# learner-shx/SVG-IR

Measured on AMD Instinct MI355X. Metric: Gaussian-surfels/sec fwd+bwd @800x800 (1 view), higher is better.
Workload: dtype f32; 1 GPU; cfg2: rgss path, P=200000 surfels, 800x800, SH degree 3, S=5, VS=0, fwd+bwd, one view per step per GPU (BASELINE.json configs[1] = cfg2 at N=1; configs[3] = cfg4, view r on rank r, at N>1); num_rendered=673008, parallelism=view-parallel x1, per_rank_cpus=not pinned

## Files before the change

### svg-ir_amd/csrc/api.hip

```cpp
#include <algorithm>
#include <cstdarg>
#include <cstdio>
#include <atomic>
#include <cstdlib>
#include <ctime>
#include <memory>
#include <mutex>
#include <string>
#include <vector>

#include "common.hpp"
#include "geom_bwd.hpp"
#include "workload_history.hpp"
#include "depth_sort_plan.hpp"

using namespace svgir;

namespace {

thread_local std::string g_err;
std::atomic<bool> g_prof{false};
WorkloadHistory g_history;
unsigned long long* pinned_words(size_t n) {
    void* ptr = nullptr;
// ... 748 lines not shown
        HIP_OK(hipMallocAsync(&redump.p, align_up((size_t)slots * seg_nstate(p->S, ra.VS) * 64 * 4), s));
        ba.seg_state = ra.seg_state = (float*)redump.p;
        g_history.count(WorkloadHistory::kRerunSlots);
        RenderArgs rd = ra;
        rd.slot_cap = (uint32_t)std::min<long long>(slots, 0xffffffffll);
        rd.dump_only = 1;
        rd.queue_order = vc.queue ? 1 : 0;
        if (launch_render_fwd(rd, svgss, s) < 0) return fail(SVGIR_ERR_INVALID, "state re-dump: no specialised composite");
        stage_mark(tm, "state_redump");
        return 0;
    }

    int clears() {
        const size_t need = svgir_backward_scratch_bytes_for(p->variant, p->P, binning_bytes, image_blob, v.W, v.H, p->S, ba.VS);
        if (!generic && (!scratch || scratch_bytes < need))
            return fail(SVGIR_ERR_INVALID, "backward scratch of %zu bytes is smaller than svgir_backward_scratch_bytes_for() = %zu",
                        scratch ? scratch_bytes : (size_t)0, need);
        clear_in_kernel = !generic && R > 0 && g->clear_base && g->clear_bytes && (((uintptr_t)g->clear_base | g->clear_bytes) & 15) == 0;
        ba.clear = clear_in_kernel ? (uint4*)g->clear_base : nullptr;
        ba.clear_n16 = clear_in_kernel ? g->clear_bytes / 16 : 0;
        if (!clear_in_kernel) {
            hipStream_t cs = generic ? s : side_stream(s);
            if (!cs) cs = s;
            hipEvent_t ev_fork = nullptr;
            if (cs != s) {
                HIP_OK(hipEventCreateWithFlags(&ev_fork, hipEventDisableTiming));
                HIP_OK(hipEventRecord(ev_fork, s));
                HIP_OK(hipStreamWaitEvent(cs, ev_fork, 0));
                (void)hipEventDestroy(ev_fork);
            }
            const size_t Pz = (size_t)p->P * 4;
            if (g->clear_base && g->clear_bytes) {
                HIP_OK(hipMemsetAsync(g->clear_base, 0, g->clear_bytes, cs));
            } else {
                struct { float* p; size_t n; } t[] = {
                    {g->dL_dmeans2D, 3 * Pz}, {g->dL_dconic, 4 * Pz}, {g->dL_dopacity, Pz}, {g->dL_dcolors, 3 * Pz},
                    {g->dL_dfeatures, (size_t)p->S * Pz}, {g->dL_dvfeatures, (size_t)ba.VS * Pz}, {g->dL_dnormal, 3 * Pz},
                    {g->dL_ddepth, Pz}, {g->dL_dmeans3D, 3 * Pz}, {g->dL_dcov3D, 6 * Pz}, {g->dL_dsh, (size_t)p->M * 3 * Pz},
                    {g->dL_dscales, 3 * Pz}, {g->dL_drotations, 4 * Pz}, {svgss ? g->dL_dviewmat : nullptr, 64},
                    {svgss ? g->dL_dprojmat : nullptr, 64}, {svgss ? g->dL_dcampos : nullptr, 12}};
                for (auto& e : t)
                    if (e.p && e.n) HIP_OK(hipMemsetAsync(e.p, 0, e.n, cs));
            }
            if (cs != s) {
                HIP_OK(hipEventCreateWithFlags(&cleared.ev, hipEventDisableTiming));
                HIP_OK(hipEventRecord(cleared.ev, cs));
            }
        }
        return 0;
    }

    int seg_build() {
        void* sc_clear = rows ? (void*)ba.row_of : (void*)ba.grad_rows;
        const size_t sc_bytes = rows ? grad_rowof_bytes(caps.cap_R) : align_up((size_t)p->P * grad_row_geom(p->S, ba.VS).RS * 4);
        bool use_list = false;
        if (R > 0) {
            if (p->shade && g->env_grad_work) shade_tabs = shade_tables(&p->shade->sp, g->env_grad_work, p->shade->sp.env_h * p->shade->sp.env_w * 3);
            use_list = g->out_weights && !generic && (p->shade || p->P >= (rows ? kListMinPRows : kListMinP));
            launch_seg_build(ra, sc_clear, sc_bytes, shade_tabs, use_list ? g->out_weights : nullptr, p->P, G.shade_work, s);
        } else if (sc_clear && !rows) {
            HIP_OK(hipMemsetAsync(sc_clear, 0, sc_bytes, s));
        }
        stage_mark(tm, "seg_build");
        if (use_list && R > 0) {
            uint32_t* cnt = G.shade_work + partition_work_words(p->P) - 1;
            launch_partition_scatter(p->P, g->out_weights, G.shade_list, G.shade_work, cnt, s);
            blended = G.shade_list; blended_n = cnt;
        }
        return 0;
    }

    void composite() {
        if (R > 0) {
            if (generic) launch_render_bwd_generic(ba, svgss, s);
            else (void)launch_render_bwd(ba, svgss, s);
        }
        stage_mark(tm, "render_bwd");
        cleared.join();
    }

    void grad_reduce() {
        if (!(R > 0 && rows)) return;
        GradReduceArgs ga;
        ga.list = blended; ga.list_count = blended_n;
        ga.P = p->P; ga.S = p->S; ga.VS = ba.VS; ga.radii = radii; ga.tiles = G.tiles; ga.rec = G.rec;
        ga.grad_rows = ba.grad_rows; ga.row_of = ba.row_of;
        ga.dL_dmean2D = g->dL_dmeans2D; ga.dL_dconic = g->dL_dconic; ga.dL_dopacity = g->dL_dopacity; ga.dL_dcolor = g->dL_dcolors;
        ga.dL_dfeature = g->dL_dfeatures; ga.dL_dvfeature = g->dL_dvfeatures; ga.dL_dnormal = g->dL_dnormal; ga.dL_ddepth = g->dL_ddepth;
        launch_grad_reduce(ga, s);
        stage_mark(tm, "grad_reduce");
    }

    int shade_backward() {
        if (!p->shade) return 0;
        const bool all = p->shade->all_surfels != 0;
        svgir_shade_params sp = p->shade->sp;
        sp.subset = nullptr; sp.subset_count = nullptr;
        if (!all) {
            if (!blended) {
                uint32_t* cnt = G.shade_work + partition_work_words(p->P) - 1;
                launch_partition(p->P, nullptr, g->out_weights, G.shade_list, G.shade_work, cnt, s);
                blended = G.shade_list; blended_n = cnt;
            }
            sp.subset = blended; sp.subset_count = blended_n;
        }
        auto in_clear = [&](const float* t, size_t floats) {
            const char* b = (const char*)g->clear_base, *q = (const char*)t;
// ... 22 lines not shown
        ga.dL_dopacity = g->dL_dopacity; ga.dL_dfeature = g->dL_dfeatures;
        ga.dL_dmean3D = g->dL_dmeans3D; ga.dL_dcov3D = g->dL_dcov3D; ga.dL_dsh = g->dL_dsh; ga.dL_dscale = g->dL_dscales;
        ga.dL_drot = g->dL_drotations; ga.dL_dviewmat = g->dL_dviewmat; ga.dL_dprojmat = g->dL_dprojmat; ga.dL_dcampos = g->dL_dcampos;
        if (ga.scales && !ga.rotations) return fail(SVGIR_ERR_INVALID, "rotations missing");
        launch_geom_bwd_blended(ga, g->out_weights, s);
        stage_mark(tm, "geom_bwd");
        hipError_t e = p->debug ? hipStreamSynchronize(s) : hipSuccess;
        if (e == hipSuccess) e = hipGetLastError();
        return e != hipSuccess ? fail(SVGIR_ERR_HIP, "backward failed: %s", hipGetErrorString(e)) : 0;
    }
};

int svgir_forward(const svgir_params* p, const svgir_outputs* o, svgir_alloc_fn geom, void* geom_ctx,
                  svgir_alloc_fn binning, void* binning_ctx, svgir_alloc_fn image, void* image_ctx, void* stream) {
    return ForwardCall::run({p, o, geom, geom_ctx, binning, binning_ctx, image, image_ctx, stream, 0}, true);
}

int svgir_forward_batch(svgir_view_call* views, int32_t count) {
    if (count < 0 || (count > 0 && !views)) return fail(SVGIR_ERR_INVALID, "views is NULL");
    std::vector<std::unique_ptr<ForwardCall>> calls;
    calls.reserve((size_t)count);
    int first_err = 0;
    for (int v = 0; v < count; v++) {
        calls.emplace_back(new ForwardCall(views[v], true));
        const int rc = calls.back()->begin();
        views[v].num_rendered = rc < 0 ? rc : 0;
        if (rc < 0 && !first_err) first_err = rc;
    }
    const std::string begin_err = first_err ? g_err : std::string();
    for (int v = 0; v < count; v++) {
        if (views[v].num_rendered < 0) continue;
        const int rc = calls[(size_t)v]->finish();
        views[v].num_rendered = rc;
        if (rc < 0 && !first_err) first_err = rc;
    }
    if (!begin_err.empty()) g_err = begin_err;
    return first_err;
}
void svgir_reset_workload_history(int32_t scope) { g_history.reset(scope); }
void svgir_speculation_stats(int64_t* out5) {
    if (out5) g_history.stats(out5);
}

size_t svgir_backward_scratch_bytes(int32_t variant, int32_t P, size_t binning_bytes, int32_t W, int32_t H, int32_t S,
                                    int32_t VS) {
    return svgir_backward_scratch_bytes_for(variant, P, binning_bytes, nullptr, W, H, S, VS);
}

size_t svgir_backward_scratch_bytes_for(int32_t variant, int32_t P, size_t binning_bytes, const char* image_blob, int32_t W, int32_t H,
                                        int32_t S, int32_t VS) {
    if (!render_specialised(S, variant == SVGIR_SVGSS ? VS : 0, variant == SVGIR_SVGSS))
        return 256;
    if (variant != SVGIR_SVGSS || VS == 0)
        return align_up((size_t)(P > 0 ? P : 1) * grad_row_geom(S, 0).RS * 4);
    ViewCounts vc;
    if (!bin_capacity(binning_bytes, image_blob, W, H, seg_nstate(S, VS), Wait::kBlock, nullptr, &vc))
        vc.cap_R = binning_capacity((long long)(binning_bytes / 48));
    if (image_blob && vc.pairs < 0) (void)hipGetLastError();
    const size_t rows = vc.pairs >= 0 ? (size_t)std::min<long long>(vc.pairs, (long long)4 * vc.cap_R) : (size_t)4 * vc.cap_R;
    return grad_scratch_bytes(vc.cap_R, rows > 0 ? rows : 1, S, VS);
}

int svgir_backward(const svgir_params* p, const svgir_grads* g, int32_t R, const int32_t* radii, char* geom_blob,
                   char* binning_blob, size_t binning_bytes, char* image_blob, char* scratch, size_t scratch_bytes,
                   void* stream) {
    return BackwardCall{p, g, R, radii, geom_blob, binning_blob, binning_bytes, image_blob, scratch, scratch_bytes, (hipStream_t)stream}.run();
}

int svgir_mark_visible(int32_t variant, int32_t P, const float* means3D, const float* viewmatrix,
                       const float* projmatrix, uint8_t* present, void* stream) {
    (void)projmatrix;
    if (P < 0) return fail(SVGIR_ERR_INVALID, "P < 0");
    if (P == 0 || variant == SVGIR_SVGSS) return 0;
    if (!means3D || !viewmatrix || !present) return fail(SVGIR_ERR_INVALID, "NULL pointer");
    launch_mark_visible(P, means3D, viewmatrix, present, (hipStream_t)stream);
    hipError_t e = hipGetLastError();
    if (e != hipSuccess) return fail(SVGIR_ERR_HIP, "mark_visible failed: %s", hipGetErrorString(e));
    return 0;
}

}
```

### svg-ir_amd/csrc/common.hpp

```cpp
#pragma once
#include <hip/hip_runtime.h>
#include <stddef.h>
#include <stdint.h>
#include <stdlib.h>

#include <algorithm>

#include "../../include/svgir_raster.h"
#include "wave.hpp"

namespace svgir {

constexpr int TILE = 16;
constexpr int BLOCK = 256;
constexpr int REC = 24;

enum RecField {
    R_X = 0, R_Y = 1, R_CX = 2, R_CY = 3,
    R_CZ = 4, R_OP = 5, R_DEPTH = 6, R_DA = 7,
    R_J0 = 8, R_J1 = 9, R_J2 = 10, R_J3 = 11,
    R_DB = 12, R_R = 13, R_G = 14, R_B = 15,
    R_NX = 16, R_NY = 17, R_NZ = 18, R_IU = 19,
    R_IV = 20, R_IBASE = 21, R_RECT = 22, R_PAD2 = 23
};
// ... 99 lines not shown

constexpr int SEG_CLASSES = 5, SEG_BLOCK_STRIDE = 8;

struct ImageLayout {
    float* final_T;
    float* final_D;
    int32_t* n_contrib;
    uint32_t* ranges;
    uint32_t* seg_block;
    uint32_t* sub_total;
    uint32_t* sub_order;
    uint32_t* sub_count;
    uint32_t* sub_ndump;
    uint32_t* sub_pair_base;
    uint32_t* sub_slot_base;
    uint32_t* counters;
    uint32_t* disp_ctr;
    uint32_t* disp_item;
    size_t ncontrib_off;
    size_t bytes;
};
constexpr int DISP_NCLS = 64, DISP_SHARDS = 8, DISP_STEP = 16;
constexpr int DISP_CTR_WORDS = DISP_NCLS * DISP_SHARDS + 2;
inline ImageLayout image_layout(char* base, int W, int H) {
    ImageLayout im;
    size_t off = 0;
    auto take = [&](size_t bytes) { char* p = base ? base + off : nullptr; off += align_up(bytes); return p; };
    const size_t N = (size_t)W * H;
    const size_t T = (size_t)((W + TILE - 1) / TILE) * ((H + TILE - 1) / TILE);
    im.final_T = (float*)take(N * 4);
    im.final_D = (float*)take(N * 4);
    im.ncontrib_off = off;
    im.n_contrib = (int32_t*)take(N * 4);
    im.ranges = (uint32_t*)take((T * 2 + (T + 255) / 256 * SEG_BLOCK_STRIDE) * 4);
    im.seg_block = im.ranges ? im.ranges + T * 2 : nullptr;
    im.sub_total = (uint32_t*)take(T * 4 * 4);
    im.sub_order = (uint32_t*)take(order_entries((W + TILE - 1) / TILE, (H + TILE - 1) / TILE) * 4);
    im.sub_count = (uint32_t*)take(T * 4 * 4);
    im.sub_ndump = (uint32_t*)take(T * 4 * 4);
    im.sub_pair_base = (uint32_t*)take(T * 4 * 4);
    im.sub_slot_base = (uint32_t*)take(T * 4 * 4);
    im.counters = (uint32_t*)take(32);
    im.disp_ctr = (uint32_t*)take(DISP_CTR_WORDS * 4);
    im.disp_item = (uint32_t*)take(order_entries((W + TILE - 1) / TILE, (H + TILE - 1) / TILE) * DISP_NCLS * 4);
    im.bytes = off;
    return im;
}

struct GradRowGeom { int NC0, P4, VS, GEO, RS; };
inline GradRowGeom grad_row_geom(int S, int VS) {
    GradRowGeom g;
    g.NC0 = 7 + S; g.P4 = (g.NC0 + 3) / 4 * 4; g.VS = VS; g.GEO = g.P4 + VS; g.RS = (g.GEO + 6 + 3) / 4 * 4;
    return g;
}
inline size_t grad_rowof_bytes(int cap) { return align_up((size_t)4 * cap * 4); }
inline size_t grad_scratch_bytes(int cap, size_t rows, int S, int VS) {
    return grad_rowof_bytes(cap) + align_up(rows * grad_row_geom(S, VS).RS * 4);
}

constexpr int SEG = 64;
#if defined(__HIPCC__)
__host__ __device__
#endif
inline uint32_t seg_slots(uint32_t total) { return total >= (uint32_t)SEG ? total / (uint32_t)SEG + 1u : 0u; }
inline size_t seg_capacity(int R, int T) { return (size_t)4 * (size_t)(R > 0 ? R : 0) / SEG + (size_t)4 * T + 1; }
constexpr int SEG_K_BITS = 14;
struct SegDesc { uint32_t sm, r0, len, count, ndump, pair_base, slot_base, pad2; };
#if defined(__HIPCC__)
__host__ __device__
#endif
inline int seg_class(uint32_t nent) { return nent >= (uint32_t)SEG ? 0 : 4 - (int)(nent * 4u / (uint32_t)SEG); }
#ifndef SEG_XCD_BLOCK_V
#define SEG_XCD_BLOCK_V 32
#endif
constexpr uint32_t SEG_XCD_BLOCK = SEG_XCD_BLOCK_V;
#if defined(__HIPCC__)
__host__ __device__
#endif
inline uint32_t seg_item_of(uint32_t w) {
    const uint32_t c = w & 7u, q = w >> 3;
    return ((q / SEG_XCD_BLOCK) * 8u + c) * SEG_XCD_BLOCK + (q % SEG_XCD_BLOCK);
}
#if defined(__HIPCC__)
__host__ __device__
#endif
inline uint32_t seg_work_ids(uint32_t n) { return (n + 8u * SEG_XCD_BLOCK - 1u) / (8u * SEG_XCD_BLOCK) * (8u * SEG_XCD_BLOCK); }

inline int binning_capacity(long long R) {
    const long long c = ((R > 0 ? R : 1) + 4095) / 4096 * 4096;
    return (int)(c > 0x7ffff000LL ? 0x7ffff000LL : c);
}

struct TileSortPlan { int bits, passes, bits_per_pass; bool single; };
constexpr int TS12_BINS = 4096, TS12_KEYS = 2048;
inline bool tile_sort_single_enabled() {
    static const bool on = [] { const char* e = getenv("SVGIR_TILE_SORT12"); return !(e && e[0] == '0'); }();
    return on;
}
inline TileSortPlan tile_sort_plan(int T) {
    int bits = 1;
    while ((1 << bits) < T) bits++;
    TileSortPlan p;
    p.bits = bits;
    p.single = T <= TS12_BINS && tile_sort_single_enabled();
    p.passes = p.single ? 1 : (bits + 7) / 8;
    p.bits_per_pass = p.single ? bits : (bits + p.passes - 1) / p.passes;
// ... 321 lines not shown
```

### svg-ir_amd/csrc/geom_bwd.hip

```cpp
#include "common.hpp"
#include "geom_bwd.hpp"

#pragma clang fp contract(off)

namespace svgir {

namespace {

struct Mat3 {
    float m[3][3];
};
__device__ __forceinline__ Mat3 mmul(const Mat3& A, const Mat3& B) {
    Mat3 r;
#pragma unroll
    for (int c = 0; c < 3; c++)
#pragma unroll
        for (int row = 0; row < 3; row++)
            r.m[c][row] = A.m[0][row] * B.m[c][0] + A.m[1][row] * B.m[c][1] + A.m[2][row] * B.m[c][2];
    return r;
}
__device__ __forceinline__ Mat3 mtr(const Mat3& A) {
    Mat3 r;
#pragma unroll
    for (int c = 0; c < 3; c++)
// ... 20 lines not shown
    int total = 0;
    {
        int cand[CHUNKS];
        bool take[CHUNKS];
#pragma unroll
        for (int c = 0; c < CHUNKS; c++) {
            const int w = blockIdx.x * GB_SPAN + c * GB_BLOCK + lane;
            const bool in_range = w < n;
            cand[c] = in_range ? (a.list ? (int)a.list[w] : w) : 0;
            take[c] = in_range && (by_weight ? weights[cand[c]] > 0.f : a.radii[cand[c]] > 0);
        }
#pragma unroll
        for (int c = 0; c < CHUNKS; c++) {
            const unsigned long long m = __ballot(take[c]);
            if (take[c]) sIdx[total + __popcll(m & ((lane == 0) ? 0ull : (~0ull >> (64 - lane))))] = cand[c];
            total += __popcll(m);
        }
    }
    if (total == 0) return;
    const bool vec = a.shs && a.M == 16 && ((((size_t)a.shs) | ((size_t)a.dL_dsh)) & 15) == 0;
    const bool coop = vec && a.D == 3;
    const int rsub = lane / 12, rpart = lane - rsub * 12;
    wave_lds_sync();
    const int npass = CHUNKS == 1 ? 1 : (total + GB_BLOCK - 1) / GB_BLOCK;
    for (int p0 = 0; p0 < npass * GB_BLOCK; p0 += GB_BLOCK) {
        const int nvis = min(GB_BLOCK, total - p0);
        const bool visible = lane < nvis;
        const int idx = visible ? sIdx[p0 + lane] : 0;
        const int* sI = sIdx + p0;
        constexpr int CR = 6;
        float4 cr[CR];
        if (coop) {
    #pragma unroll
            for (int j = 0; j < CR; j++) {
                const int r = 5 * j + rsub;
                cr[j] = (rsub < 5 && r < nvis) ? reinterpret_cast<const float4*>(a.shs)[(size_t)sI[r] * 12 + rpart]
                                              : make_float4(0.f, 0.f, 0.f, 0.f);
            }
        }
        const bool surface = cfg_flag(a.cfg, 0);
        const bool lrn_cam = a.svgss && a.cfg.len >= 0 && cfg_flag(a.cfg, 3);
        float V[16], PR[16], campos[3] = {0.f, 0.f, 0.f};
        float in_color[3] = {0.f, 0.f, 0.f}, in_normal[3] = {0.f, 0.f, 0.f}, in_depth = 0.f, in_m2d[2] = {0.f, 0.f}, in_conic[3] = {0.f, 0.f, 0.f}, in_opacity = 0.f;
        float mean[3] = {0.f, 0.f, 0.f}, c3[6] = {0.f, 0.f, 0.f, 0.f, 0.f, 0.f};
        float4 qq = make_float4(0.f, 0.f, 0.f, 0.f);
        float sc_in[3] = {0.f, 0.f, 0.f};
        uint32_t cm = 0;
        if (visible) {
    #pragma unroll
        for (int i = 0; i < 16; i++) { V[i] = a.view[i]; PR[i] = a.proj[i]; }
        if (a.shs) { campos[0] = a.campos[0]; campos[1] = a.campos[1]; campos[2] = a.campos[2]; }

        if (a.packed) {
            const int P4 = (7 + a.S + 3) / 4 * 4, RS = (P4 + 6 + 3) / 4 * 4;
            const float* row = a.packed + (size_t)idx * RS;
            const float4 h0 = reinterpret_cast<const float4*>(row)[0], h1 = reinterpret_cast<const float4*>(row)[1];
            const float4 t0 = reinterpret_cast<const float4*>(row + P4)[0], t1 = reinterpret_cast<const float4*>(row + P4)[1];
            in_color[0] = h0.x; in_color[1] = h0.y; in_color[2] = h0.z; in_normal[0] = h0.w; in_normal[1] = h1.x; in_normal[2] = h1.y;
            in_depth = h1.z;
            in_m2d[0] = t0.x; in_m2d[1] = t0.y; in_conic[0] = t0.z; in_conic[1] = t0.w; in_conic[2] = t1.x;
            in_opacity = t1.y;
        } else {
    #pragma unroll
            for (int c = 0; c < 3; c++) { in_color[c] = a.dL_dcolor[3 * idx + c]; in_normal[c] = a.dL_dnormal[3 * idx + c]; }
            in_depth = a.dL_ddepth[idx];
            in_m2d[0] = a.dL_dmean2D[3 * idx]; in_m2d[1] = a.dL_dmean2D[3 * idx + 1];
            in_conic[0] = a.dL_dconic[4 * idx]; in_conic[1] = a.dL_dconic[4 * idx + 1]; in_conic[2] = a.dL_dconic[4 * idx + 3];
        }
        mean[0] = a.means3D[3 * idx]; mean[1] = a.means3D[3 * idx + 1]; mean[2] = a.means3D[3 * idx + 2];
    #pragma unroll
        for (int i = 0; i < 6; i++) c3[i] = a.cov3D[6 * idx + i];
        if (a.shs) cm = a.clamped[idx];
        if (a.scales) {
            qq = reinterpret_cast<const float4*>(a.rotations)[idx];
    #pragma unroll
            for (int i = 0; i < 3; i++) sc_in[i] = a.scales[3 * idx + i];
        }
        }
        if (coop) {
    #pragma unroll
            for (int j = 0; j < CR; j++) {
                const int r = 5 * j + rsub;
                if (rsub < 5 && r < nvis) sRow[r][rpart] = cr[j];
            }
            for (int r0 = 5 * CR; r0 < nvis; r0 += 5) {
                const int r = r0 + rsub;
                if (rsub < 5 && r < nvis)
                    sRow[r][rpart] = reinterpret_cast<const float4*>(a.shs)[(size_t)sI[r] * 12 + rpart];
            }
        }
        if (visible) {
        const int nk = (a.D + 1) * (a.D + 1);
        float sh[48];
        if (a.shs) {
            const float* shp = a.shs + (size_t)idx * a.M * 3;
            if (coop) {
                wave_lds_sync();
    #pragma unroll
                for (int i = 0; i < 12; i++) {
                    const float4 v = sRow[lane][i];
                    sh[4 * i] = v.x; sh[4 * i + 1] = v.y; sh[4 * i + 2] = v.z; sh[4 * i + 3] = v.w;
                }
            } else if (vec) {
    #pragma unroll
                for (int i = 0; i < 12; i++) {
                    const float4 v = reinterpret_cast<const float4*>(shp)[i];
                    sh[4 * i] = v.x; sh[4 * i + 1] = v.y; sh[4 * i + 2] = v.z; sh[4 * i + 3] = v.w;
                }
            } else {
    #pragma unroll
                for (int i = 0; i < 48; i++) sh[i] = i < 3 * nk ? shp[i] : 0.f;
            }
        }
        if (a.packed) {
            const int P4 = (7 + a.S + 3) / 4 * 4, RS = (P4 + 6 + 3) / 4 * 4;
            const float* row = a.packed + (size_t)idx * RS;
            for (int c = 0; c < a.S; c++) a.dL_dfeature[(size_t)idx * a.S + c] = row[7 + c];
        }
        float dmean[3];
        float dcv[6];

        {
            const float dcon[3] = {in_conic[0], in_conic[1], in_conic[2]};
            float t[3] = {V[0] * mean[0] + V[4] * mean[1] + V[8] * mean[2] + V[12],
                          V[1] * mean[0] + V[5] * mean[1] + V[9] * mean[2] + V[13],
                          V[2] * mean[0] + V[6] * mean[1] + V[10] * mean[2] + V[14]};
            const float limx = 1.3f * a.tanx, limy = 1.3f * a.tany;
            const float txtz = t[0] / t[2], tytz = t[1] / t[2];
            t[0] = fminf(limx, fmaxf(-limx, txtz)) * t[2];
            t[1] = fminf(limy, fmaxf(-limy, tytz)) * t[2];
            const float xgm = (txtz < -limx || txtz > limx) ? 0.f : 1.f;
            const float ygm = (tytz < -limy || tytz > limy) ? 0.f : 1.f;
            const float hx = a.focal_x, hy = a.focal_y;
            const float J0 = hx / t[2], J1 = -(hx * t[0]) / (t[2] * t[2]), J2 = hy / t[2], J3 = -(hy * t[1]) / (t[2] * t[2]);
            Mat3 Jm, Wm, Vk;
            Jm.m[0][0] = J0; Jm.m[0][1] = 0.f; Jm.m[0][2] = J1;
            Jm.m[1][0] = 0.f; Jm.m[1][1] = J2; Jm.m[1][2] = J3;
            Jm.m[2][0] = 0.f; Jm.m[2][1] = 0.f; Jm.m[2][2] = 0.f;
            Wm.m[0][0] = V[0]; Wm.m[0][1] = V[4]; Wm.m[0][2] = V[8];
            Wm.m[1][0] = V[1]; Wm.m[1][1] = V[5]; Wm.m[1][2] = V[9];
            Wm.m[2][0] = V[2]; Wm.m[2][1] = V[6]; Wm.m[2][2] = V[10];
            Vk.m[0][0] = c3[0]; Vk.m[0][1] = c3[1]; Vk.m[0][2] = c3[2];
            Vk.m[1][0] = c3[1]; Vk.m[1][1] = c3[3]; Vk.m[1][2] = c3[4];
            Vk.m[2][0] = c3[2]; Vk.m[2][1] = c3[4]; Vk.m[2][2] = c3[5];
            const Mat3 Tm = mmul(Wm, Jm);
            const Mat3 cov = mmul(mmul(mtr(Tm), mtr(Vk)), Tm);
            const float ca = cov.m[0][0] + 0.3f, cb = cov.m[0][1], cc = cov.m[1][1] + 0.3f;
            const float denom = ca * cc - cb * cb;
            float da = 0.f, db = 0.f, dc = 0.f;
            const float d2i = 1.0f / ((denom * denom) + 0.0000001f);
    #define TC(i, j) Tm.m[i][j]
    #define VC_(i, j) Vk.m[i][j]
            if (d2i != 0) {
                da = d2i * (-cc * cc * dcon[0] + 2 * cb * cc * dcon[1] + (denom - ca * cc) * dcon[2]);
                dc = d2i * (-ca * ca * dcon[2] + 2 * ca * cb * dcon[1] + (denom - ca * cc) * dcon[0]);
                db = d2i * 2 * (cb * cc * dcon[0] - (denom + 2 * cb * cb) * dcon[1] + ca * cb * dcon[2]);
                dcv[0] = (TC(0, 0) * TC(0, 0) * da + TC(0, 0) * TC(1, 0) * db + TC(1, 0) * TC(1, 0) * dc);
                dcv[3] = (TC(0, 1) * TC(0, 1) * da + TC(0, 1) * TC(1, 1) * db + TC(1, 1) * TC(1, 1) * dc);
                dcv[5] = (TC(0, 2) * TC(0, 2) * da + TC(0, 2) * TC(1, 2) * db + TC(1, 2) * TC(1, 2) * dc);
                dcv[1] = 2 * TC(0, 0) * TC(0, 1) * da + (TC(0, 0) * TC(1, 1) + TC(0, 1) * TC(1, 0)) * db + 2 * TC(1, 0) * TC(1, 1) * dc;
                dcv[2] = 2 * TC(0, 0) * TC(0, 2) * da + (TC(0, 0) * TC(1, 2) + TC(0, 2) * TC(1, 0)) * db + 2 * TC(1, 0) * TC(1, 2) * dc;
                dcv[4] = 2 * TC(0, 2) * TC(0, 1) * da + (TC(0, 1) * TC(1, 2) + TC(0, 2) * TC(1, 1)) * db + 2 * TC(1, 1) * TC(1, 2) * dc;
            } else {
    #pragma unroll
                for (int i = 0; i < 6; i++) dcv[i] = 0.f;
            }
            const float dT00 = 2 * (TC(0, 0) * VC_(0, 0) + TC(0, 1) * VC_(0, 1) + TC(0, 2) * VC_(0, 2)) * da +
                               (TC(1, 0) * VC_(0, 0) + TC(1, 1) * VC_(0, 1) + TC(1, 2) * VC_(0, 2)) * db;
            const float dT01 = 2 * (TC(0, 0) * VC_(1, 0) + TC(0, 1) * VC_(1, 1) + TC(0, 2) * VC_(1, 2)) * da +
// ... 221 lines not shown
```

### svg-ir_amd/csrc/render_bwd_plain.hip

```cpp
#include <algorithm>

#include "common.hpp"
#include "stage.hpp"
#include "dev_trace.hpp"

namespace svgir {

namespace {

typedef const __attribute__((address_space(4))) float cfloat;
typedef const __attribute__((address_space(4))) uint32_t cuint;

#ifndef BWDP_GRID_MULT
#define BWDP_GRID_MULT 4
#endif
#ifndef BWDP_WPE
#define BWDP_WPE 4
#endif

template <int S>
struct PlainGeom {
    static constexpr int SB = 8;
    static constexpr int NC0 = 7 + S;
    static constexpr int GROW = NC0 + 1;
    static constexpr int PS = 68;
    static constexpr int PROWS = 24;
    static constexpr size_t off_m = (size_t)PROWS * PS * 4;
    static constexpr size_t off_c = off_m + (size_t)SB * 8 * 4;
    static constexpr size_t off_q = off_c + (size_t)3 * SB * 16;
    static constexpr size_t lds_bytes = off_q + (size_t)SEG * 8;
    static_assert(NC0 <= 16, "one 16-wide MFMA column tile");
    static_assert((size_t)64 * GROW * 4 <= off_m, "the G transposition tile aliases the panel");
};

template <int S, bool SVGSS>
__global__ void __launch_bounds__(64) __attribute__((amdgpu_waves_per_eu(BWDP_WPE, BWDP_WPE)))
render_bwd_plain_kernel(const RenderBwdArgs a) {
    using PG = PlainGeom<S>;
    constexpr int SB = PG::SB, NC0 = PG::NC0, GROW = PG::GROW, PS = PG::PS;
    constexpr int SS = S > 0 ? S : 1;
    constexpr int P4 = (NC0 + 3) / 4 * 4, GEO = P4, RS = (GEO + 6 + 3) / 4 * 4;
    extern __shared__ __attribute__((aligned(16))) char smem[];
    float* sP = reinterpret_cast<float*>(smem);
    float* sG = sP;
    float* sM = reinterpret_cast<float*>(smem + PG::off_m);
    float4* sC = reinterpret_cast<float4*>(smem + PG::off_c);
    uint2* sQ = reinterpret_cast<uint2*>(smem + PG::off_q);

    const int lane = threadIdx.x;
    const bool surface = cfg_flag(a.cfg, 0), normalize_depth = cfg_flag(a.cfg, 1);
    const bool sp = surface && cfg_flag(a.cfg, 2);
    const bool bgeom = SVGSS ? true : (a.backward_geometry != 0);
    const size_t N_ = (size_t)a.W * a.H;
    const float ddelx_dx = 0.5f * a.W, ddely_dy = 0.5f * a.H;
    const int colB = lane & 15, grpB = lane >> 4;

    float cx0, cx1, cx2, momy[2];
    {
        const int ex = colB == 1 || colB == 4 ? 1 : colB == 3 ? 2 : 0;
        const int ey = colB == 2 || colB == 4 ? 1 : colB == 5 ? 2 : 0;
        cx0 = (colB < 6 && ex == 0) ? 1.f : 0.f; cx1 = ex == 1 ? 1.f : 0.f; cx2 = ex == 2 ? 1.f : 0.f;
#pragma unroll
        for (int h = 0; h < 2; h++) {
            const float my = (float)(2 * grpB + h) - 3.5f;
            momy[h] = ey == 0 ? 1.f : ey == 1 ? my : my * my;
        }
    }

    typedef const __attribute__((address_space(4))) uint32_t cu32;
    cu32* dsc0 = (cu32*)(uintptr_t)(a.seg_desc + min(seg_item_of(blockIdx.x), (uint32_t)a.seg_cap));
    uint32_t d_sm = dsc0[0], d_r0 = dsc0[1], d_len = dsc0[2], d_count = dsc0[3], d_ndump = dsc0[4], d_sb = dsc0[6];
    if (a.clear) {
        const uint4 z = make_uint4(0u, 0u, 0u, 0u);
        for (size_t i = (size_t)blockIdx.x * 64 + threadIdx.x; i < a.clear_n16; i += (size_t)gridDim.x * 64) a.clear[i] = z;
    }
    const uint32_t nlive = min(a.seg_count[0], (uint32_t)a.seg_cap);
    const uint32_t nwork = seg_work_ids(nlive);
    if (blockIdx.x >= nwork) return;
    DEV_TRACE_DECL();
    [[maybe_unused]] unsigned dev_items = 0, dev_cands = 0;
    for (uint32_t w = blockIdx.x; w < nwork; w += gridDim.x) {
    const uint32_t item = seg_item_of(w);
    if (item >= nlive) continue;
    if (w != blockIdx.x) {
        cu32* dsc = (cu32*)(uintptr_t)(a.seg_desc + item);
        d_sm = dsc[0]; d_r0 = dsc[1]; d_len = dsc[2]; d_count = dsc[3]; d_ndump = dsc[4]; d_sb = dsc[6];
    }
    wave_lds_sync();
    const uint32_t sm = d_sm, r0 = d_r0, tlen = d_len;
    const int count = (int)d_count, ndump = (int)d_ndump;
    const int sid = (int)(sm >> SEG_K_BITS), kseg = (int)(sm & ((1u << SEG_K_BITS) - 1u));
    const int tile = sid >> 2, sub = sid & 3;
    const int seg_lo = kseg * SEG, seg_hi = min(count, seg_lo + SEG);
    if (seg_hi <= seg_lo) continue;
// ... 57 lines not shown
    for (int i = 0; i < 3; i++) { gC[i] = (inside && a.g_color) ? a.g_color[i * N_ + pid] : 0.f; gN[i] = (inside && a.g_normal) ? a.g_normal[i * N_ + pid] : 0.f; }
#pragma unroll
    for (int i = 0; i < SS; i++) gF[i] = (inside && i < S && a.g_feature) ? a.g_feature[i * N_ + pid] : 0.f;
    if (inside) { gD = a.g_depth ? a.g_depth[pid] : 0.f; gO = a.g_opacity ? a.g_opacity[pid] : 0.f; }
    const float bgdot = a.bg[0] * gC[0] + a.bg[1] * gC[1] + a.bg[2] * gC[2];
    const float omt = 1.f - T_final;
    const float gDn = normalize_depth ? gD / omt : gD;
    const float kdn = normalize_depth ? -gD * D_final * T_final / (omt * omt) : 0.f;
    const float gO_kbg = gO - (bgdot + (normalize_depth ? 0.f : 10.f * gD));
    const float q5g = sp ? -gD : 0.f;

    uint32_t wmax = last_contributor;
    wmax = wave_reduce_max(wmax);
    if (wmax == 0) continue;

    float T = T_final;
    float last_alpha = 0.f;
    float A_acc = 0.f, s_last = 0.f;
    if (kseg < ndump) {
        constexpr int NST = 8 + S;
        const uint32_t sbase = d_sb;
        const float* e = a.seg_state + ((size_t)(sbase + kseg) * NST) * 64 + lane;
        const float* f = a.seg_state + ((size_t)(sbase + ndump) * NST) * 64 + lane;
        T = e[0];
        float dot = (f[7 * 64] - e[7 * 64]) * gDn;
#pragma unroll
        for (int i = 0; i < 3; i++) {
            dot += (f[(1 + i) * 64] - e[(1 + i) * 64]) * gC[i];
            dot += (f[(4 + i) * 64] - e[(4 + i) * 64]) * gN[i];
        }
        if (bgeom) {
#pragma unroll
            for (int i = 0; i < S; i++) dot += (f[(8 + i) * 64] - e[(8 + i) * 64]) * gF[i];
        }
        A_acc = dot * __builtin_amdgcn_rcpf(T);
    }

    {
        float* g = sG + lane * GROW;
        g[0] = gC[0]; g[1] = gC[1]; g[2] = gC[2];
        g[3] = surface ? gN[0] * 10.f : 0.f; g[4] = surface ? gN[1] * 10.f : 0.f; g[5] = surface ? gN[2] * 10.f : 0.f;
        g[6] = gDn;
#pragma unroll
        for (int i = 0; i < S; i++) g[7 + i] = gF[i];
    }
    float Bp[16];
    wave_lds_sync();
    {
        const float* gB = sG + (16 * grpB) * GROW + (colB < NC0 ? colB : 0);
#pragma unroll
        for (int kk = 0; kk < 16; kk++) Bp[kk] = colB < NC0 ? gB[kk * GROW] : 0.f;
    }
    wave_lds_sync();

    int nskip = 0;
    {
        uint2 e = make_uint2(0u, 0u);
        if (lane < nent) e = sub_in[seg_hi - 1 - lane];
        sQ[lane] = e;
        nskip = __popcll(__ballot(lane < nent && e.y >= wmax));
    }
    const float gNe0 = surface ? gN[0] : 0.f, gNe1 = surface ? gN[1] : 0.f, gNe2 = surface ? gN[2] : 0.f;
    float gFe[SS];
#pragma unroll
    for (int i = 0; i < SS; i++) gFe[i] = bgeom ? gF[i] : 0.f;
    const float spf = sp ? 1.f : 0.f;
    const float gOT = gO_kbg * T_final;

    const int cstart = (nskip / SB) * SB;
    Cand cur = spec_cur;
    Entry en1 = spec_en1;
    if (cstart != 0) {
        cur = fetch_rec(fetch_entry(cstart));
        en1 = fetch_entry(cstart + 1);
    }
    auto prefetch_consts = [&](int cb) {
        int lC = lane;
        asm volatile("" : "+v"(lC));
        if (lC < 3 * SB) {
            const int cq = lC & 7, chunk = lC >> 3;
            const uint32_t gq = sQ[min(cb + cq, SEG - 1)].x;
            const float* src = a.rec + (uint32_t)(gq * (uint32_t)REC + (uint32_t)(chunk == 2 ? 12 : 4 * chunk));
            __builtin_amdgcn_global_load_lds(src, (__attribute__((address_space(3))) void*)(smem + PG::off_c), 16, 0, 0);
        }
    };
    wave_lds_sync();
    prefetch_consts(cstart);
    DEV_TRACE_MARK(0);
    dev_items++; dev_cands += (unsigned)nent;
    for (int c0 = cstart; c0 < nent; c0 += SB) {
        uint32_t live = 0;
        float hw = 0.f, hv = 0.f, hu = 0.f;
#pragma unroll
        for (int k = 0; k < SB; k++) {
            const Cand nxt = fetch_rec(en1);
            en1 = fetch_entry(c0 + k + 2);
            const float dx = cur.X - pxf, dy = cur.Y - pyf;
            if (k > 0) {
                sP[(k - 1) * PS + lane] = hw; sP[(SB + k - 1) * PS + lane] = hv; sP[(2 * SB + k - 1) * PS + lane] = hu;
            }
            const float pw = pair_power(cur.cxx, cur.cxy, cur.cyy, dx, dy);
            const float Gs = exp_nonpos(pw);
            const float al = fminf(0.99f, cur.op * Gs);
            const bool pre = cur.slot < last_contributor && pw <= 0.0f && al >= (1.0f / 255.0f);
            const float ioma = __builtin_amdgcn_rcpf(1.f - al);
            float sd = cur.cr * gC[0] + cur.cg * gC[1] + cur.cb * gC[2];
            sd += cur.nx * gNe0 + cur.ny * gNe1 + cur.nz * gNe2;
            const float d_cur = cur.dep - spf * (dx * cur.DA + dy * cur.DB);
            sd += d_cur * gDn;
#pragma unroll
            for (int ch = 0; ch < S; ch++) sd += cur.f[ch] * gFe[ch];
            const float inv_Told = __builtin_amdgcn_rcpf(T);
            const float Tn = T * ioma;
            const float An = last_alpha * s_last + (1.f - last_alpha) * A_acc;
            float dL_dalpha = kdn * inv_Told + (sd - An);
            dL_dalpha *= Tn;
            dL_dalpha += gOT * ioma;
            T = pre ? Tn : T;
            A_acc = pre ? An : A_acc;
            s_last = pre ? sd : s_last;
            last_alpha = pre ? al : last_alpha;
            hw = pre ? al * Tn : 0.f;
            hv = pre ? Gs * dL_dalpha : 0.f;
            hu = pre ? q5g : 0.f;
            live |= (__builtin_amdgcn_ballot_w64(pre) != 0ull ? 1u : 0u) << k;
            cur = nxt;
        }
        sP[(SB - 1) * PS + lane] = hw; sP[(2 * SB - 1) * PS + lane] = hv; sP[(3 * SB - 1) * PS + lane] = hu;
        DEV_TRACE_MARK(2);
        if (live != 0) {
        wave_lds_sync();
        int lB = lane;
        asm volatile("" : "+v"(lB));
        const int colB = lB & 15, grpB = lB >> 4;
        f32x4 accM = {0.f, 0.f, 0.f, 0.f};
        {
            const float4* ap = reinterpret_cast<const float4*>(sP + (SB + colB) * PS + 16 * grpB);
            const float4 a0 = ap[0], a1 = ap[1], a2 = ap[2], a3 = ap[3];
            const float av[16] = {a0.x, a0.y, a0.z, a0.w, a1.x, a1.y, a1.z, a1.w,
                                  a2.x, a2.y, a2.z, a2.w, a3.x, a3.y, a3.z, a3.w};
            float c0l = cx0;
            asm volatile("" : "+v"(c0l));
#pragma unroll
            for (int kk = 0; kk < 16; kk++) {
                const float mx = (float)(kk & 7) - 3.5f;
                accM = __builtin_amdgcn_mfma_f32_16x16x4f32(av[kk], (c0l + mx * (cx1 + mx * cx2)) * momy[kk >> 3], accM, 0, 0, 0);
            }
        }
        if (grpB < 2) {
            if (colB < 6) {
#pragma unroll
                for (int rr = 0; rr < 4; rr++) sM[(4 * grpB + rr) * 8 + colB] = accM[rr];
            }
        } else if (colB == 0) {
#pragma unroll
            for (int rr = 0; rr < 4; rr++) sM[(4 * (grpB - 2) + rr) * 8 + 6] = accM[rr];
        }
        f32x4 accP = {0.f, 0.f, 0.f, 0.f};
        {
            const float4* ap = reinterpret_cast<const float4*>(sP + colB * PS + 16 * grpB);
            const float4 a0 = ap[0], a1 = ap[1], a2 = ap[2], a3 = ap[3];
            const float av[16] = {a0.x, a0.y, a0.z, a0.w, a1.x, a1.y, a1.z, a1.w,
                                  a2.x, a2.y, a2.z, a2.w, a3.x, a3.y, a3.z, a3.w};
#pragma unroll
            for (int kk = 0; kk < 16; kk++) accP = __builtin_amdgcn_mfma_f32_16x16x4f32(av[kk], Bp[kk], accP, 0, 0, 0);
        }
        __builtin_amdgcn_s_waitcnt(0x0f70);
        wave_lds_sync();
        DEV_TRACE_MARK(3);
        {
            const int cq = lB & 7, jq = lB >> 3;
            if (jq < 6 && ((live >> cq) & 1u)) {
                const float4 m03 = *reinterpret_cast<const float4*>(sM + cq * 8);
                const float4 m47 = *reinterpret_cast<const float4*>(sM + cq * 8 + 4);
                const float4 Aq = sC[cq], Bq = sC[SB + cq];
                const float DBq = sC[2 * SB + cq].x;
                const float Xc = Aq.x - cxs, Yc = Aq.y - cys;
                const float M0 = m03.x, M1 = m03.y, M2 = m03.z, M3 = m03.w, M4 = m47.x, M5 = m47.y, Q = m47.z;
                const float Sx = Xc * M0 - M1, Sy = Yc * M0 - M2;
                const float hf = Bq.y * -0.5f;
                float ge;
                if (jq == 0) ge = hf * 2.f * (Aq.z * Sx + Aq.w * Sy) * ddelx_dx + Q * Bq.w;
                else if (jq == 1) ge = hf * 2.f * (Bq.x * Sy + Aq.w * Sx) * ddely_dy + Q * DBq;
                else if (jq == 2) ge = hf * (Xc * (Sx - M1) + M3);
                else if (jq == 3) ge = hf * ((Xc * Sy - Yc * M1) + M4);
                else if (jq == 4) ge = hf * (Yc * (Sy - M2) + M5);
                else ge = M0;
                if (ge != 0.f) atomic_add_f32(a.grad_rows + (uint32_t)(sQ[c0 + cq].x * (uint32_t)RS + (uint32_t)(GEO + jq)), ge);
            }
        }
        if (grpB < 2) {
#pragma unroll
            for (int rr = 0; rr < 4; rr++) {
                const int cB = 4 * grpB + rr;
                const bool mine = ((live >> cB) & 1u) && colB < NC0 && accP[rr] != 0.f;
                if (mine) atomic_add_f32(a.grad_rows + (uint32_t)(sQ[c0 + cB].x * (uint32_t)RS + (uint32_t)colB), accP[rr]);
            }
        }
        wave_lds_sync();
        }
        if (c0 + SB < nent) prefetch_consts(c0 + SB);
        DEV_TRACE_MARK(1);
    }
    }
    DEV_TRACE_END(1, dev_items, dev_cands, blockIdx.x);
}

template <int S, bool SVGSS>
void launch(const RenderBwdArgs& a, hipStream_t s) {
    using PG = PlainGeom<S>;
    const int grid = std::max(8, std::min(a.seg_cap, BWDP_GRID_MULT * 256 * 4 * BWDP_WPE) & ~7);
    hipLaunchKernelGGL((render_bwd_plain_kernel<S, SVGSS>), dim3(grid), dim3(64), PG::lds_bytes, s, a);
}

}

int launch_render_bwd_plain(const RenderBwdArgs& a, bool svgss, hipStream_t s) {
    if (a.VS != 0) return -1;
#define CASE(SV, SG) if (a.S == SV && svgss == SG) { launch<SV, SG>(a, s); return 0; }
    CASE(0, true) CASE(5, true) CASE(0, false) CASE(5, false) CASE(3, false) CASE(1, false)
#undef CASE
    return -1;
}

#if defined(SVGIR_DEV)
extern "C" int svgir_dev_trace_read_bwd_plain(unsigned long long* out, int cap_records) {
    unsigned int n[2];
    if (hipMemcpyFromSymbol(n, HIP_SYMBOL(svgir::g_dev_trace_n), sizeof(n)) != hipSuccess) return -1;
    int cnt = (int)std::min<unsigned>(n[1], (unsigned)std::min(cap_records, svgir::DEV_TRACE_CAP));
    if (cnt > 0 && hipMemcpyFromSymbol(out, HIP_SYMBOL(svgir::g_dev_trace), (size_t)cnt * svgir::DEV_TRACE_WORDS * 8,
                                       (size_t)svgir::DEV_TRACE_CAP * svgir::DEV_TRACE_WORDS * 8) != hipSuccess) return -1;
    n[1] = 0;
    (void)hipMemcpyToSymbol(HIP_SYMBOL(svgir::g_dev_trace_n), n, sizeof(n));
    return cnt;
}
#endif

}
```

Measured before the change: 630.4 million surfels/s.

## Batch color-gradient MFMA over two segment chunks and centralize packed row geometry

The color/feature gradient MFMA in the plain backward render kernel now runs once per pair of SB-sized chunks. It double-buffers the weight rows in LDS (PROWS raised from 24 to 32) and tracks a combined 16-bit liveness mask, so all 16 MFMA rows do useful work instead of half being padding. This cuts MFMA issues, LDS reads and sync points per chunk, in exchange for more LDS and extra zeroing of the second buffer. It also adds a packed_row_geom helper with an optional 16/32 alignment mode (off by default) and an optional split-accumulator MFMA variant (off by default).

```diff
diff --git a/svg-ir_amd/csrc/api.hip b/svg-ir_amd/csrc/api.hip
--- a/svg-ir_amd/csrc/api.hip
+++ b/svg-ir_amd/csrc/api.hip
@@ -824,7 +824,7 @@
 
     int seg_build() {
         void* sc_clear = rows ? (void*)ba.row_of : (void*)ba.grad_rows;
-        const size_t sc_bytes = rows ? grad_rowof_bytes(caps.cap_R) : align_up((size_t)p->P * grad_row_geom(p->S, ba.VS).RS * 4);
+        const size_t sc_bytes = rows ? grad_rowof_bytes(caps.cap_R) : align_up((size_t)p->P * packed_row_geom(p->S).RS * 4);
         bool use_list = false;
         if (R > 0) {
             if (p->shade && g->env_grad_work) shade_tabs = shade_tables(&p->shade->sp, g->env_grad_work, p->shade->sp.env_h * p->shade->sp.env_w * 3);
@@ -953,7 +953,7 @@
     if (!render_specialised(S, variant == SVGIR_SVGSS ? VS : 0, variant == SVGIR_SVGSS))
         return 256;
     if (variant != SVGIR_SVGSS || VS == 0)
-        return align_up((size_t)(P > 0 ? P : 1) * grad_row_geom(S, 0).RS * 4);
+        return align_up((size_t)(P > 0 ? P : 1) * packed_row_geom(S).RS * 4);
     ViewCounts vc;
     if (!bin_capacity(binning_bytes, image_blob, W, H, seg_nstate(S, VS), Wait::kBlock, nullptr, &vc))
         vc.cap_R = binning_capacity((long long)(binning_bytes / 48));
diff --git a/svg-ir_amd/csrc/common.hpp b/svg-ir_amd/csrc/common.hpp
--- a/svg-ir_amd/csrc/common.hpp
+++ b/svg-ir_amd/csrc/common.hpp
@@ -175,6 +175,14 @@
     GradRowGeom g;
     g.NC0 = 7 + S; g.P4 = (g.NC0 + 3) / 4 * 4; g.VS = VS; g.GEO = g.P4 + VS; g.RS = (g.GEO + 6 + 3) / 4 * 4;
     return g;
+}
+#ifndef PACKED_ROW_ALIGNED
+#define PACKED_ROW_ALIGNED 0
+#endif
+struct PackedRowGeom { int NC0, GEO, RS; };
+constexpr PackedRowGeom packed_row_geom(int S) {
+    const int NC0 = 7 + S, P4 = (NC0 + 3) / 4 * 4, RC = (P4 + 6 + 3) / 4 * 4;
+    return (!PACKED_ROW_ALIGNED || RC <= 16 || P4 > 16) ? PackedRowGeom{NC0, P4, RC} : PackedRowGeom{NC0, 16, 32};
 }
 inline size_t grad_rowof_bytes(int cap) { return align_up((size_t)4 * cap * 4); }
 inline size_t grad_scratch_bytes(int cap, size_t rows, int S, int VS) {
diff --git a/svg-ir_amd/csrc/geom_bwd.hip b/svg-ir_amd/csrc/geom_bwd.hip
--- a/svg-ir_amd/csrc/geom_bwd.hip
+++ b/svg-ir_amd/csrc/geom_bwd.hip
@@ -96,10 +96,10 @@
         if (a.shs) { campos[0] = a.campos[0]; campos[1] = a.campos[1]; campos[2] = a.campos[2]; }
 
         if (a.packed) {
-            const int P4 = (7 + a.S + 3) / 4 * 4, RS = (P4 + 6 + 3) / 4 * 4;
-            const float* row = a.packed + (size_t)idx * RS;
+            const PackedRowGeom rg = packed_row_geom(a.S);
+            const float* row = a.packed + (size_t)idx * rg.RS;
             const float4 h0 = reinterpret_cast<const float4*>(row)[0], h1 = reinterpret_cast<const float4*>(row)[1];
-            const float4 t0 = reinterpret_cast<const float4*>(row + P4)[0], t1 = reinterpret_cast<const float4*>(row + P4)[1];
+            const float4 t0 = reinterpret_cast<const float4*>(row + rg.GEO)[0], t1 = reinterpret_cast<const float4*>(row + rg.GEO)[1];
             in_color[0] = h0.x; in_color[1] = h0.y; in_color[2] = h0.z; in_normal[0] = h0.w; in_normal[1] = h1.x; in_normal[2] = h1.y;
             in_depth = h1.z;
             in_m2d[0] = t0.x; in_m2d[1] = t0.y; in_conic[0] = t0.z; in_conic[1] = t0.w; in_conic[2] = t1.x;
@@ -157,8 +157,7 @@
             }
         }
         if (a.packed) {
-            const int P4 = (7 + a.S + 3) / 4 * 4, RS = (P4 + 6 + 3) / 4 * 4;
-            const float* row = a.packed + (size_t)idx * RS;
+            const float* row = a.packed + (size_t)idx * packed_row_geom(a.S).RS;
             for (int c = 0; c < a.S; c++) a.dL_dfeature[(size_t)idx * a.S + c] = row[7 + c];
         }
         float dmean[3];
diff --git a/svg-ir_amd/csrc/render_bwd_plain.hip b/svg-ir_amd/csrc/render_bwd_plain.hip
--- a/svg-ir_amd/csrc/render_bwd_plain.hip
+++ b/svg-ir_amd/csrc/render_bwd_plain.hip
@@ -17,6 +17,9 @@
 #ifndef BWDP_WPE
 #define BWDP_WPE 4
 #endif
+#ifndef BWDP_MFMA_ACC
+#define BWDP_MFMA_ACC 1
+#endif
 
 template <int S>
 struct PlainGeom {
@@ -24,7 +27,7 @@
     static constexpr int NC0 = 7 + S;
     static constexpr int GROW = NC0 + 1;
     static constexpr int PS = 68;
-    static constexpr int PROWS = 24;
+    static constexpr int PROWS = 32;
     static constexpr size_t off_m = (size_t)PROWS * PS * 4;
     static constexpr size_t off_c = off_m + (size_t)SB * 8 * 4;
     static constexpr size_t off_q = off_c + (size_t)3 * SB * 16;
@@ -39,7 +42,7 @@
     using PG = PlainGeom<S>;
     constexpr int SB = PG::SB, NC0 = PG::NC0, GROW = PG::GROW, PS = PG::PS;
     constexpr int SS = S > 0 ? S : 1;
-    constexpr int P4 = (NC0 + 3) / 4 * 4, GEO = P4, RS = (GEO + 6 + 3) / 4 * 4;
+    constexpr int GEO = packed_row_geom(S).GEO, RS = packed_row_geom(S).RS;
     extern __shared__ __attribute__((aligned(16))) char smem[];
     float* sP = reinterpret_cast<float*>(smem);
     float* sG = sP;
@@ -203,6 +206,8 @@
         for (int kk = 0; kk < 16; kk++) Bp[kk] = colB < NC0 ? gB[kk * GROW] : 0.f;
     }
     wave_lds_sync();
+#pragma unroll
+    for (int k = 0; k < SB; k++) sP[(SB + k) * PS + lane] = 0.f;
 
     int nskip = 0;
     {
@@ -239,7 +244,10 @@
     prefetch_consts(cstart);
     DEV_TRACE_MARK(0);
     dev_items++; dev_cands += (unsigned)nent;
+    uint32_t live16 = 0;
     for (int c0 = cstart; c0 < nent; c0 += SB) {
+        const int par = ((c0 - cstart) / SB) & 1;
+        float* sPw = sP + par * (SB * PS) + lane;
         uint32_t live = 0;
         float hw = 0.f, hv = 0.f, hu = 0.f;
 #pragma unroll
@@ -248,7 +256,7 @@
             en1 = fetch_entry(c0 + k + 2);
             const float dx = cur.X - pxf, dy = cur.Y - pyf;
             if (k > 0) {
-                sP[(k - 1) * PS + lane] = hw; sP[(SB + k - 1) * PS + lane] = hv; sP[(2 * SB + k - 1) * PS + lane] = hu;
+                sPw[(k - 1) * PS] = hw; sP[(2 * SB + k - 1) * PS + lane] = hv; sP[(3 * SB + k - 1) * PS + lane] = hu;
             }
             const float pw = pair_power(cur.cxx, cur.cxy, cur.cyy, dx, dy);
             const float Gs = exp_nonpos(pw);
@@ -277,7 +285,7 @@
             live |= (__builtin_amdgcn_ballot_w64(pre) != 0ull ? 1u : 0u) << k;
             cur = nxt;
         }
-        sP[(SB - 1) * PS + lane] = hw; sP[(2 * SB - 1) * PS + lane] = hv; sP[(3 * SB - 1) * PS + lane] = hu;
+        sPw[(SB - 1) * PS] = hw; sP[(3 * SB - 1) * PS + lane] = hv; sP[(4 * SB - 1) * PS + lane] = hu;
         DEV_TRACE_MARK(2);
         if (live != 0) {
         wave_lds_sync();
@@ -286,17 +294,20 @@
         const int colB = lB & 15, grpB = lB >> 4;
         f32x4 accM = {0.f, 0.f, 0.f, 0.f};
         {
-            const float4* ap = reinterpret_cast<const float4*>(sP + (SB + colB) * PS + 16 * grpB);
+            const float4* ap = reinterpret_cast<const float4*>(sP + (2 * SB + colB) * PS + 16 * grpB);
             const float4 a0 = ap[0], a1 = ap[1], a2 = ap[2], a3 = ap[3];
             const float av[16] = {a0.x, a0.y, a0.z, a0.w, a1.x, a1.y, a1.z, a1.w,
                                   a2.x, a2.y, a2.z, a2.w, a3.x, a3.y, a3.z, a3.w};
             float c0l = cx0;
             asm volatile("" : "+v"(c0l));
+            f32x4 accM2 = {0.f, 0.f, 0.f, 0.f};
 #pragma unroll
             for (int kk = 0; kk < 16; kk++) {
                 const float mx = (float)(kk & 7) - 3.5f;
-                accM = __builtin_amdgcn_mfma_f32_16x16x4f32(av[kk], (c0l + mx * (cx1 + mx * cx2)) * momy[kk >> 3], accM, 0, 0, 0);
-            }
+                f32x4& acc = (BWDP_MFMA_ACC == 2 && (kk & 1)) ? accM2 : accM;
+                acc = __builtin_amdgcn_mfma_f32_16x16x4f32(av[kk], (c0l + mx * (cx1 + mx * cx2)) * momy[kk >> 3], acc, 0, 0, 0);
+            }
+            if (BWDP_MFMA_ACC == 2) accM += accM2;
         }
         if (grpB < 2) {
             if (colB < 6) {
@@ -306,15 +317,6 @@
         } else if (colB == 0) {
 #pragma unroll
             for (int rr = 0; rr < 4; rr++) sM[(4 * (grpB - 2) + rr) * 8 + 6] = accM[rr];
-        }
-        f32x4 accP = {0.f, 0.f, 0.f, 0.f};
-        {
-            const float4* ap = reinterpret_cast<const float4*>(sP + colB * PS + 16 * grpB);
-            const float4 a0 = ap[0], a1 = ap[1], a2 = ap[2], a3 = ap[3];
-            const float av[16] = {a0.x, a0.y, a0.z, a0.w, a1.x, a1.y, a1.z, a1.w,
-                                  a2.x, a2.y, a2.z, a2.w, a3.x, a3.y, a3.z, a3.w};
-#pragma unroll
-            for (int kk = 0; kk < 16; kk++) accP = __builtin_amdgcn_mfma_f32_16x16x4f32(av[kk], Bp[kk], accP, 0, 0, 0);
         }
         __builtin_amdgcn_s_waitcnt(0x0f70);
         wave_lds_sync();
@@ -340,15 +342,36 @@
                 if (ge != 0.f) atomic_add_f32(a.grad_rows + (uint32_t)(sQ[c0 + cq].x * (uint32_t)RS + (uint32_t)(GEO + jq)), ge);
             }
         }
-        if (grpB < 2) {
+        wave_lds_sync();
+        }
+        live16 = par ? (live16 | (live << SB)) : live;
+        if ((par || c0 + SB >= nent) && live16 != 0) {
+            wave_lds_sync();
+            int lP = lane;
+            asm volatile("" : "+v"(lP));
+            const int colP = lP & 15, grpP = lP >> 4;
+            f32x4 accP = {0.f, 0.f, 0.f, 0.f};
+            {
+                const float4* ap = reinterpret_cast<const float4*>(sP + colP * PS + 16 * grpP);
+                const float4 a0 = ap[0], a1 = ap[1], a2 = ap[2], a3 = ap[3];
+                const float av[16] = {a0.x, a0.y, a0.z, a0.w, a1.x, a1.y, a1.z, a1.w,
+                                      a2.x, a2.y, a2.z, a2.w, a3.x, a3.y, a3.z, a3.w};
+                f32x4 accP2 = {0.f, 0.f, 0.f, 0.f};
+#pragma unroll
+                for (int kk = 0; kk < 16; kk++) {
+                    f32x4& acc = (BWDP_MFMA_ACC == 2 && (kk & 1)) ? accP2 : accP;
+                    acc = __builtin_amdgcn_mfma_f32_16x16x4f32(av[kk], Bp[kk], acc, 0, 0, 0);
+                }
+                if (BWDP_MFMA_ACC == 2) accP += accP2;
+            }
+            const int cp0 = c0 - par * SB;
 #pragma unroll
             for (int rr = 0; rr < 4; rr++) {
-                const int cB = 4 * grpB + rr;
-                const bool mine = ((live >> cB) & 1u) && colB < NC0 && accP[rr] != 0.f;
-                if (mine) atomic_add_f32(a.grad_rows + (uint32_t)(sQ[c0 + cB].x * (uint32_t)RS + (uint32_t)colB), accP[rr]);
-            }
-        }
-        wave_lds_sync();
+                const int cB = 4 * grpP + rr;
+                const bool mine = ((live16 >> cB) & 1u) && colP < NC0 && accP[rr] != 0.f;
+                if (mine) atomic_add_f32(a.grad_rows + (uint32_t)(sQ[cp0 + cB].x * (uint32_t)RS + (uint32_t)colP), accP[rr]);
+            }
+            wave_lds_sync();
         }
         if (c0 + SB < nent) prefetch_consts(c0 + SB);
         DEV_TRACE_MARK(1);
```

Result: faster. 641.5 million surfels/s, median of 6 (+1.8%).
